# DavidHan008/SLAM-1

Hardware: AMD Instinct MI355X
Metric: frames/sec tracking+local-BA @1280x720 (higher is better)
Workload: dtype u8+f32+f64

## Files before the change

### include/slam355.h

```cpp
#ifndef SLAM355_H
#define SLAM355_H

#include <stddef.h>
#include <stdint.h>

#ifdef __cplusplus
extern "C" {
#endif

#define SLAM355_ABI_VERSION 1

#define SLAM_OK 0
#define SLAM_ERR_ARG (-1)
#define SLAM_ERR_HIP (-2)
#define SLAM_ERR_WORKSPACE (-3)
#define SLAM_ERR_COMM (-4)

int slam_abi_version(void);
const char* slam_last_error(void);
int slam_device_count(void);

int slam_hamming_knn2(const uint8_t* d_q, const int32_t* d_nq, int q_cap,
                      const uint8_t* d_t, const int32_t* d_nt, int t_cap,
                      int batch, int32_t* d_idx2, int32_t* d_dist2,
// ... 142 lines not shown
  double* delta_c;
  double* red_part;
  double* small;
  double* state;
  uint32_t* ticket;
  const int32_t* sg_ptr;
  const int32_t* sg_meta;
  const int32_t* obs_meta;
  const int32_t* chk_optr;
  const int32_t* chk_cptr;
  const int32_t* bslot_ab;
  const int32_t* tl_sched;
  const int32_t* tl_sched_host;
  int32_t* asm_tab;
  const int32_t* asm_act;
  int32_t n_asm_act;
  int32_t loss;
  double loss_scale;
  const uint32_t* cam_fixed;
} slam_ba_problem;
int slam_ba_problem_size(void);

#define SLAM_TL_FLOW_MAX_T 256

#ifndef SLAM_BA_MAX_BATCH
#define SLAM_BA_MAX_BATCH 16
#endif

enum {
  SLAM_PLAN_PERM = 0,
  SLAM_PLAN_ORDER,
  SLAM_PLAN_OBS_CAM, SLAM_PLAN_OBS_PT, SLAM_PLAN_PT_PTR, SLAM_PLAN_GRP_PTR,
  SLAM_PLAN_GRP_CSLOT, SLAM_PLAN_CSLOT_CAM, SLAM_PLAN_GRP_BSLOT, SLAM_PLAN_BSLOT_BLK,
  SLAM_PLAN_BLOCKS, SLAM_PLAN_CAM_CSLOT_PTR, SLAM_PLAN_CSLOT_ROW, SLAM_PLAN_BLK_BSLOT_PTR,
  SLAM_PLAN_BSLOT_ROW, SLAM_PLAN_SG_PTR, SLAM_PLAN_SG_META, SLAM_PLAN_SG_CAMS,
  SLAM_PLAN_OBS_LA, SLAM_PLAN_CHK_COBS, SLAM_PLAN_OBS_META, SLAM_PLAN_CHK_OPTR,
  SLAM_PLAN_CHK_CPTR, SLAM_PLAN_BSLOT_AB,
  SLAM_PLAN_NTAB
};
typedef struct slam_ba_plan_info {
  int32_t ok, n_obs, n_grps, n_sgrps, n_cslots, n_bslots, n_blocks, chunks_per_wg;
  long long off[SLAM_PLAN_NTAB], len[SLAM_PLAN_NTAB];
  long long total;
} slam_ba_plan_info;
long long slam_ba_plan_bound(int n_cams, int n_pts, int n_obs, int n_block_list);
int slam_ba_plan_mfma(int n_cams, int n_pts, int n_obs, const int32_t* cam_idx,
                      const int32_t* pt_idx, const int32_t* block_list, int n_block_list,
                      int chunks_per_wg, int32_t* out, long long out_cap,
                      slam_ba_plan_info* info);

#define SLAM_STAGE_NF64 17
#define SLAM_STAGE_META (12 + SLAM_STAGE_NF64 + SLAM_PLAN_NTAB)
int slam_ba_stage_windows(int n_win, int n, int cap, const double* rows, const int32_t* cnt,
                          const double* maps, int map_cap, const int32_t* M, const double* cams,
                          double u_off, double v_off, double* h64, long long cap64, int32_t* h32,
                          long long cap32, const void* d64, const void* d32,
                          slam_ba_problem* probs, long long* meta, long long* need);

int slam_ba_red_slots(int n_grps);
long long slam_ba_chol_len(int n_cams, const int32_t* tl_sched_host);
long long slam_ba_sys_len(int n_cams, int n_blocks);

int slam_ba_build_system(const slam_ba_problem* prob, void* stream);
int slam_ba_solve_step(const slam_ba_problem* prob, void* stream);
int slam_ba_decide(const slam_ba_problem* prob, void* stream);
int slam_ba_iterate(const slam_ba_problem* prob, int n_iter, void* stream);
int slam_ba_reset(const slam_ba_problem* prob, double lambda0, void* stream);
int slam_ba_iterate_batch(const slam_ba_problem* probs, int n_probs, int n_iter, void* stream);

long long slam_ba_cov_workspace_len(int n_cams);
int slam_ba_covariance(const slam_ba_problem* prob, const int32_t* d_pairs, int n_pairs,
                       double rank_tol, double* d_cov, double* d_ws, long long ws_len,
                       int32_t* d_status, void* stream);

int slam_ba_covariance_points(const slam_ba_problem* prob,
                              const int32_t* d_pairs, int n_pairs, double* d_cov,
                              const int32_t* d_points, int n_points, double* d_cov_pp,
                              const int32_t* d_cross, int n_cross, double* d_cov_pc,
                              double rank_tol, double* d_ws, long long ws_len,
                              int32_t* d_status , void* stream);

int slam_ba_set_solve_lds_floor(int bytes);

int slam_orb_set_lds_floor(int bytes);

int slam_orb_set_corner_cap(int entries_per_wave);

int slam_count_min(const int32_t* d_count, int n, int32_t* d_min, void* stream);
int slam_ba_reset_batch(const slam_ba_problem* probs, int n_probs, double lambda0, void* stream);

#define SLAM_COMM_ID_BYTES 128
typedef struct slam_comm_opaque* slam_comm_t;
int slam_comm_unique_id(void* h_id);
int slam_comm_init(int nranks, int rank, const void* h_id, slam_comm_t* comm);
int slam_comm_destroy(slam_comm_t comm);
int slam_comm_allreduce_f64(slam_comm_t comm, double* d_buf, long long n, void* stream);
int slam_ba_step_distributed(const slam_ba_problem* prob, slam_comm_t comm, void* stream);


int slam_pose_chain_objective(const double* params, int n_vec, int n_frames, int loop,
                              double* resid, void* stream);
long long slam_pose_chain_workspace_len(int n_frames);
int slam_pose_chain_trf(double* ws, int n_frames, int loop, int max_iter, int first, double ftol,
                        double xtol, double gtol, int max_nfev, double* state, void* stream);

typedef struct slam_pg_problem {
  int32_t n_poses, n_edges;
  int32_t loss;
  int32_t sched_len;
  double loss_scale;
  double* poses[2];
  const int32_t* edge_ij;
  const int32_t* edge_ij_host;
  const double* meas;
  const double* sqrt_info;
  const uint32_t* pose_fixed;
  const int32_t* sched;
  const int32_t* sched_host;
  double* ws;
  long long ws_len;
  double* state;
} slam_pg_problem;
int slam_pg_problem_size(void);
long long slam_pg_workspace_len(int n_poses, int n_edges, int n_tiles_stored);
int slam_pg_reset(const slam_pg_problem* prob, double lambda0, void* stream);
int slam_pg_iterate(const slam_pg_problem* prob, int n_iters, void* stream);
int slam_pg_residual(const slam_pg_problem* prob, double* d_e, double* d_r, void* stream);
int slam_pg_jacobian(const slam_pg_problem* prob, double* d_Ji, double* d_Jj, void* stream);

long long slam_pg_cov_workspace_len(int n_poses, int n_cols);
int slam_pg_covariance(const slam_pg_problem* prob, const int32_t* d_pairs, const int32_t* pairs_host,
                       int n_pairs, double rank_tol, double* d_cov ,
                       double* d_ws, long long ws_len, int32_t* d_status, void* stream);
int slam_pg_gate(const slam_pg_problem* prob, const int32_t* d_cand_ij, const int32_t* cand_ij_host,
                 const double* d_meas, const double* d_sqrt_info , int n_cand,
                 double rank_tol, double* d_d2, double* d_P, double* d_e ,
                 double* d_ws, long long ws_len, int32_t* d_status , void* stream);


int slam_bow_histograms(const uint8_t* desc, const int32_t* count, int n_each, int n_img, int cap,
                        const double* centers, int n_clusters, int32_t* labels, int32_t* hist,
                        void* stream);
int slam_bow_query(const int32_t* qhist, int n_query, const int32_t* db, const int32_t* n_db,
                   int n_clusters, int32_t* idx, double* val, void* stream);
int slam_bow_lloyd(const uint8_t* X, int n_points, double* centers, double* centers_tmp,
                   int n_clusters, int n_iter, int32_t* labels, double* shift, void* stream);


int slam_fast_tiles_workspace_bytes(int batch, int H, int W, int tile_h, int tile_w, int per_tile,
                                    size_t* bytes);
int slam_fast_tiles(const uint8_t* d_img, int batch, int H, int W, int stride, int tile_h,
                    int tile_w, int threshold, int per_tile, void* d_ws, size_t ws_bytes,
                    float* d_kp, int32_t* d_count, int kp_cap, void* stream);

int slam_lk_pyramid_layout(int H, int W, int win, int max_level, int* nlev, size_t* img_bytes);
int slam_lk_build_pyramids(const uint8_t* d_img, int n_img, int H, int W, int stride, int win,
                           int max_level, uint8_t* d_pyr, int16_t* d_deriv, void* stream);
int slam_lk_track(const uint8_t* d_prev_pyr, const int16_t* d_prev_deriv, const uint8_t* d_next_pyr,
                  long long pair_stride_imgs, int batch, int H, int W, int win, int max_level,
                  int max_count, double eps, float min_eig, const float* d_pts, int pts_stride,
                  const int32_t* d_npts, int cap, float* d_out, uint8_t* d_status, float* d_err,
                  void* stream);
int slam_lk_filter(const float* d_p1, int p1_stride, const float* d_p2, const uint8_t* d_status,
                   const float* d_err, const int32_t* d_npts, int cap, int batch, int H, int W,
                   float max_error, int lower_bounds, float* d_tp1, float* d_tp2, int32_t* d_idx,
                   int32_t* d_count, void* stream);
// ... 23 lines not shown
```

### slam-1_amd/csrc/ba.hip

```cpp
#include "ba_common.hpp"
#include "ba_epilogue.hpp"
#include "ba_layout.hpp"
#include "ba_project.hpp"
#include "dpp_fmac.hpp"

using slam::Launch;
using slam::launch_build;
using slam::make_launch;

namespace {

constexpr double kLamMin = 1e-16, kLamMax = 1e32;

#ifndef SLAM_BA_XCD
#define SLAM_BA_XCD 1
#endif
__device__ __forceinline__ int2 ba_xcd_map() {
  const int gx = (int)gridDim.x, n = (int)gridDim.y;
  if (!SLAM_BA_XCD || n < 8 || (n & 7)) return int2{(int)blockIdx.x, (int)blockIdx.y};
  const int lin = (int)blockIdx.y * gx + (int)blockIdx.x;
  const int xcd = lin & 7, slot = lin >> 3;
  const int wi = slot / gx;
  return int2{slot - wi * gx, xcd + 8 * wi};
}
// ... 1129 lines not shown
int check_problem(const slam_ba_problem* p) {
  SLAM_REQUIRE(p != nullptr, "slam_ba: null problem");
  SLAM_REQUIRE(p->n_cams > 0 && p->n_pts >= 0 && p->n_obs >= 0, "slam_ba: bad sizes");
  SLAM_REQUIRE(p->loss >= 0 && p->loss <= 3,
               "slam_ba: loss %d (0 linear, 1 huber, 2 soft_l1, 3 cauchy)", p->loss);
  SLAM_REQUIRE(p->loss == 0 || (std::isfinite(p->loss_scale) && p->loss_scale > 0.0),
               "slam_ba: loss %d needs a finite loss_scale > 0, not %g", p->loss, p->loss_scale);
  SLAM_REQUIRE(p->cams[0] && p->cams[1] && p->camrec[0] && p->camrec[1] &&
                   p->cpart && p->bpart && p->grp_ptr && p->grp_cslot && p->grp_bslot &&
                   p->cslot_obs_ptr && p->bslot_pair_ptr && p->cam_cslot_ptr && p->cslot_row && p->bslot_row &&
                   p->blk_bslot_ptr && p->blocks && p->ticket && p->sys && p->state &&
                   p->small && p->red_part && p->delta_c,
               "slam_ba: null buffer");
  SLAM_REQUIRE(p->n_grps >= 1, "slam_ba: n_grps must be >= 1 (an empty group for P = 0)");
  SLAM_REQUIRE(p->lin_mode == 0 || p->lin_mode == 1, "slam_ba: lin_mode must be 0 or 1");
  SLAM_REQUIRE(p->chk_optr != nullptr, "slam_ba: chk_optr (= pt_ptr[grp_ptr]) required");
  SLAM_REQUIRE(p->lin_mode == 0 || (p->n_sgrps >= 1 && p->sg_ptr && p->sg_meta && p->obs_meta &&
                                     p->chk_cptr && p->bslot_ab),
               "slam_ba: lin_mode 1 needs n_sgrps >= 1 and the supergroup tables");
  SLAM_REQUIRE(sys_packed(p->n_cams) ? (p->n_blocks >= p->n_cams &&
                                        p->n_blocks <= p->n_cams * (p->n_cams + 1) / 2)
                                     : p->n_blocks == p->n_cams * (p->n_cams + 1) / 2,
               "slam_ba: n_blocks must list all C(C+1)/2 upper blocks (9C <= %d) or the "
               "diagonal and every block with common points (packed)", kDenseMaxN);
  SLAM_REQUIRE(!p->tl_sched == !p->tl_sched_host,
               "slam_ba: tl_sched and tl_sched_host come together");
  SLAM_REQUIRE(p->asm_act == nullptr ||
                   (sys_packed(p->n_cams) && p->asm_tab == nullptr && p->n_asm_act >= 1 &&
                    p->n_asm_act <= p->n_blocks),
               "slam_ba: asm_act (n_asm_act %d of %d blocks) needs a packed system without asm_tab",
               p->n_asm_act, p->n_blocks);
  SLAM_REQUIRE(p->tl_mode == 0 || p->tl_mode == 1, "slam_ba: tl_mode must be 0 or 1");
  SLAM_REQUIRE(!sys_packed(p->n_cams) || p->chol != nullptr,
               "slam_ba: chol workspace (slam_ba_chol_len doubles) required for 9C > %d",
               kLdsMaxN);
  SLAM_REQUIRE(!sys_packed(p->n_cams) || p->tl_sched != nullptr,
               "slam_ba: the tile schedule (tl_sched, ba.tl_schedule) is required for 9C > %d",
               kLdsMaxN);
  return SLAM_OK;
}

}

extern "C" int slam_ba_red_slots(int n_grps) { return 2 * n_grps; }

extern "C" int slam_ba_problem_size(void) { return (int)sizeof(slam_ba_problem); }

extern "C" long long slam_ba_sys_len(int n_cams, int n_blocks) {
  const long long c9 = 9ll * n_cams;
  return sys_vec_off(n_cams, n_blocks) + 3 * c9 + n_cams;
}

extern "C" int slam_ba_residual(const double* d_cams, const double* d_pts,
                                const int32_t* d_cam_idx, const int32_t* d_pt_idx,
                                const double* d_qs, int n_obs, double* d_resid, void* stream) {
  SLAM_REQUIRE(n_obs >= 0, "slam_ba_residual: n_obs < 0");
  if (n_obs == 0) return SLAM_OK;
  SLAM_REQUIRE(d_cams && d_pts && d_cam_idx && d_pt_idx && d_qs && d_resid,
               "slam_ba_residual: null pointer");
  k_residual<<<nblk(n_obs, kBS), kBS, 0, slam::as_stream(stream)>>>(
      d_cams, d_pts, d_cam_idx, d_pt_idx, d_qs, n_obs, d_resid, nullptr);
  SLAM_LAUNCHED("k_residual");
  return SLAM_OK;
}

extern "C" int slam_ba_jacobian(const double* d_cams, const double* d_pts,
                                const int32_t* d_cam_idx, const int32_t* d_pt_idx,
                                const double* d_qs, int n_obs, double* d_resid, double* d_jac,
                                void* stream) {
  SLAM_REQUIRE(n_obs >= 0, "slam_ba_jacobian: n_obs < 0");
  if (n_obs == 0) return SLAM_OK;
  SLAM_REQUIRE(d_cams && d_pts && d_cam_idx && d_pt_idx && d_qs && d_resid && d_jac,
               "slam_ba_jacobian: null pointer");
  k_residual<<<nblk(n_obs, kBS), kBS, 0, slam::as_stream(stream)>>>(
      d_cams, d_pts, d_cam_idx, d_pt_idx, d_qs, n_obs, d_resid, d_jac);
  SLAM_LAUNCHED("k_residual(jac)");
  return SLAM_OK;
}

namespace {

static size_t g_solve_lds_floor = 0;

static int launch_reset(const Launch& L, double lam0, hipStream_t s) {
  k_reset<<<dim3(1, L.n), 64, 0, s>>>(L.b, lam0);
  SLAM_LAUNCHED("k_reset");
  return SLAM_OK;
}

}

int slam::make_launch(const slam_ba_problem* probs, int n, Launch* L) {
  SLAM_REQUIRE(n >= 1 && n <= kBaMaxBatch, "slam_ba: batch of %d problems (1..%d)", n, kBaMaxBatch);
  SLAM_REQUIRE(probs != nullptr, "slam_ba: null problem array");
  L->n = n;
  L->max_grps = L->max_blocks = L->max_sgrps = 0;
  L->mode = probs[0].lin_mode;
  L->solve_lds = 0;
  L->dense = true;
  L->robust = false;
  for (int i = 0; i < n; ++i) {
    if (int rc = check_problem(probs + i)) return rc;
    for (int j = 0; j < i; ++j)
      SLAM_REQUIRE(probs[j].state != probs[i].state && probs[j].sys != probs[i].sys,
                   "slam_ba: problems %d and %d of a batch share buffers", j, i);
    SLAM_REQUIRE(probs[i].lin_mode == L->mode,
                 "slam_ba: problems of one batch must share lin_mode");
    L->b.p[i] = probs[i];
    L->max_grps = max(L->max_grps, probs[i].n_grps);
    L->max_sgrps = max(L->max_sgrps, probs[i].n_sgrps);
    L->max_blocks = max(L->max_blocks, probs[i].asm_act != nullptr ? probs[i].n_asm_act : probs[i].n_blocks);
    L->solve_lds = std::max(L->solve_lds, slam::solve_blk_lds(probs[i].n_cams));
    L->solve_lds = std::max(L->solve_lds, g_solve_lds_floor);
    L->dense = L->dense && !sys_packed(probs[i].n_cams);
    L->robust = L->robust || probs[i].loss != 0;
  }
  SLAM_REQUIRE(n == 1 || L->dense,
               "slam_ba: batched problems must use the one-workgroup solver (9C <= %d)", kLdsMaxN);
  return SLAM_OK;
}

int slam::launch_build(const Launch& L, hipStream_t s) {
  bool folded = L.mode == 1;
  for (int i = 0; i < L.n; ++i) folded = folded && L.b.p[i].asm_tab != nullptr;
  if (L.mode == 1) {
    if (L.robust) k_lin_mfma<true><<<dim3(L.max_sgrps, L.n), kMWG, 0, s>>>(L.b);
    else k_lin_mfma<false><<<dim3(L.max_sgrps, L.n), kMWG, 0, s>>>(L.b);
    SLAM_LAUNCHED("k_lin_mfma");
  } else {
    if (L.robust) k_linearize<true><<<dim3(L.max_grps, L.n), kLinWG, 0, s>>>(L.b);
    else k_linearize<false><<<dim3(L.max_grps, L.n), kLinWG, 0, s>>>(L.b);
    SLAM_LAUNCHED("k_linearize");
  }
  if (!folded) {
    k_assemble<<<dim3(L.max_blocks, L.n), kAsmWG, 0, s>>>(L.b);
    SLAM_LAUNCHED("k_assemble");
  }
  return SLAM_OK;
}

namespace {

static int launch_solve(const Launch& L, bool fuse_decide, hipStream_t s) {
  if (int rc = L.dense ? slam::launch_solve_blk(L, s) : slam::launch_solve_tiled(L.b.p[0], s)) return rc;
  if (L.robust) {
    if (fuse_decide) k_back_trial<true, true><<<dim3(L.max_grps, L.n), kGrp, 0, s>>>(L.b);
    else k_back_trial<false, true><<<dim3(L.max_grps, L.n), kGrp, 0, s>>>(L.b);
  } else if (fuse_decide) {
    k_back_trial<true, false><<<dim3(L.max_grps, L.n), kGrp, 0, s>>>(L.b);
  } else {
    k_back_trial<false, false><<<dim3(L.max_grps, L.n), kGrp, 0, s>>>(L.b);
  }
  SLAM_LAUNCHED("k_back_trial");
  return SLAM_OK;
}

}

extern "C" int slam_ba_set_solve_lds_floor(int bytes) {
  SLAM_REQUIRE(bytes >= 0 && bytes <= 160 * 1024, "slam_ba_set_solve_lds_floor: %d B", bytes);
  g_solve_lds_floor = (size_t)bytes;
  return SLAM_OK;
}

extern "C" int slam_ba_reset(const slam_ba_problem* prob, double lambda0, void* stream) {
  return slam_ba_reset_batch(prob, 1, lambda0, stream);
}

extern "C" int slam_ba_reset_batch(const slam_ba_problem* probs, int n_probs, double lambda0,
                                   void* stream) {
  SLAM_REQUIRE(n_probs >= 0, "slam_ba_reset_batch: n_probs < 0");
  SLAM_REQUIRE(n_probs == 0 || probs != nullptr, "slam_ba_reset_batch: null problem array");
  for (int i0 = 0; i0 < n_probs; i0 += kBaMaxBatch) {
    Launch L;
    const int n = min(kBaMaxBatch, n_probs - i0);
    for (int i = 0; i < n; ++i)
      if (int rc = check_problem(probs + i0 + i)) return rc;
    L.n = n;
    for (int i = 0; i < n; ++i) L.b.p[i] = probs[i0 + i];
    if (int rc = launch_reset(L, lambda0, slam::as_stream(stream))) return rc;
  }
  return SLAM_OK;
}

extern "C" int slam_ba_build_system(const slam_ba_problem* prob, void* stream) {
  Launch L;
  if (int rc = make_launch(prob, 1, &L)) return rc;
  return launch_build(L, slam::as_stream(stream));
}

extern "C" int slam_ba_solve_step(const slam_ba_problem* prob, void* stream) {
  Launch L;
  if (int rc = make_launch(prob, 1, &L)) return rc;
  return launch_solve(L, false, slam::as_stream(stream));
}

extern "C" int slam_ba_decide(const slam_ba_problem* prob, void* stream) {
  Launch L;
  if (int rc = make_launch(prob, 1, &L)) return rc;
  k_decide<<<dim3(1, 1), 64, 0, slam::as_stream(stream)>>>(L.b);
  SLAM_LAUNCHED("k_decide");
  return SLAM_OK;
}

extern "C" int slam_ba_iterate(const slam_ba_problem* prob, int n_iter, void* stream) {
  return slam_ba_iterate_batch(prob, 1, n_iter, stream);
}

extern "C" int slam_ba_iterate_batch(const slam_ba_problem* probs, int n_probs, int n_iter,
                                     void* stream) {
  SLAM_REQUIRE(n_probs >= 0 && n_iter >= 0, "slam_ba_iterate_batch: negative count");
  SLAM_REQUIRE(n_probs == 0 || probs != nullptr, "slam_ba_iterate_batch: null problem array");
  hipStream_t s = slam::as_stream(stream);
  int i0 = 0;
  while (i0 < n_probs) {
    int n = 0;
    while (n < kBaMaxBatch && i0 + n < n_probs && (n == 0 || !sys_packed(probs[i0 + n].n_cams)) &&
           !(n > 0 && sys_packed(probs[i0].n_cams)))
      ++n;
    Launch L;
    if (int rc = make_launch(probs + i0, n, &L)) return rc;
    for (int it = 0; it < n_iter; ++it) {
      if (int rc = launch_build(L, s)) return rc;
      if (int rc = launch_solve(L, true, s)) return rc;
    }
    i0 += n;
  }
  return SLAM_OK;
}

#ifdef SLAM_LINM_PROFILE
extern "C" int slam_linm_stamps(unsigned long long* out, int n) {
  SLAM_HIP(hipDeviceSynchronize());
  SLAM_HIP(hipMemcpyFromSymbol(out, HIP_SYMBOL(g_linm_stamp), (size_t)n * 8 * sizeof(unsigned long long)));
  return SLAM_OK;
}
#endif
```

### slam-1_amd/csrc/ba_common.hpp

```cpp
#pragma once

#include "common.hpp"

#include <cmath>

namespace {

typedef double d4 __attribute__((ext_vector_type(4)));

constexpr double kDiagMin = 1e-6, kDiagMax = 1e32;

constexpr int kBaMaxBatch = SLAM_BA_MAX_BATCH;
struct BaBatch {
  slam_ba_problem p[kBaMaxBatch];
};
#define BA_PROB(b) const slam_ba_problem& p = (b).p[blockIdx.y]
static_assert(sizeof(slam_ba_problem) == 408, "slam_ba_problem grew: re-check the kernarg size");
static_assert(sizeof(BaBatch) <= 16 * 408, "BaBatch kernel argument size");

__device__ __forceinline__ void lm_wave_priority() { __builtin_amdgcn_s_setprio(3); }

__device__ __forceinline__ double block_sum(double v, double* lds) {
  for (int off = 32; off > 0; off >>= 1) v += __shfl_down(v, off, 64);
  const int lane = threadIdx.x & 63, wid = threadIdx.x >> 6;
  if (lane == 0) lds[wid] = v;
  __syncthreads();
  double s = 0.0;
  if (threadIdx.x == 0) {
    const int nw = (blockDim.x + 63) >> 6;
    for (int w = 0; w < nw; ++w) s += lds[w];
  }
  __syncthreads();
  return s;
}

__device__ __forceinline__ int cur_of(const double* state) {
  return state[SLAM_BA_ST_CUR] != 0.0 ? 1 : 0;
}

__device__ __forceinline__ double clampd(double d) { return fmin(fmax(d, kDiagMin), kDiagMax); }

constexpr int kDenseMaxN = 120;
__host__ __device__ __forceinline__ bool sys_packed(int n_cams) { return 9 * n_cams > kDenseMaxN; }
__host__ __device__ __forceinline__ long long sys_vec_off(int n_cams, int n_blocks) {
  return sys_packed(n_cams) ? 81ll * n_blocks : 81ll * n_cams * n_cams;
}
constexpr int kLdsMaxN = kDenseMaxN;

__device__ __forceinline__ void st_sc1(double* p, double v) {
  __hip_atomic_store(p, v, __ATOMIC_RELAXED, __HIP_MEMORY_SCOPE_AGENT);
}
__device__ __forceinline__ double ld_sc1(const double* p) {
  return __hip_atomic_load(const_cast<double*>(p), __ATOMIC_RELAXED, __HIP_MEMORY_SCOPE_AGENT);
}
__device__ __forceinline__ unsigned ticket_add(uint32_t* p) {
  return __hip_atomic_fetch_add(p, 1u, __ATOMIC_RELAXED, __HIP_MEMORY_SCOPE_AGENT);
}
__device__ __forceinline__ void ticket_reset(uint32_t* p) {
  __hip_atomic_store(p, 0u, __ATOMIC_RELAXED, __HIP_MEMORY_SCOPE_AGENT);
}

constexpr int kBS = 256;

}

namespace slam {

struct Launch {
  BaBatch b;
  int n, max_grps, max_blocks, max_sgrps, mode;
  size_t solve_lds;
  bool dense;
  bool robust;
};

size_t solve_blk_lds(int n_cams);
int launch_solve_blk(const Launch& L, hipStream_t s);
int launch_solve_tiled(const slam_ba_problem& p, hipStream_t s);
int make_launch(const slam_ba_problem* probs, int n, Launch* L);
int launch_build(const Launch& L, hipStream_t s);

}
```

### slam-1_amd/csrc/ba_solve.hip

```cpp
#include "ba_common.hpp"
#include "ba_epilogue.hpp"
#include "dpp_fmac.hpp"

namespace {

constexpr int kSolveHdr = 32;

#ifdef SLAM_SOLVE_PROFILE
#define SOLVE_PROF_T(i) uint64_t prof_t##i = wall_clock64()
#define SOLVE_PROF_END()                                                        \
  do {                                                                          \
    const uint64_t prof_e = wall_clock64();                                     \
    if (threadIdx.x == 0) {                                                     \
      p.state[12] = 10.0 * (double)(prof_t1 - prof_t0);                         \
      p.state[13] = 10.0 * (double)(prof_t2 - prof_t1);                         \
      p.state[14] = 10.0 * (double)(prof_t3 - prof_t2);                         \
      p.state[15] = 10.0 * (double)(prof_e - prof_t3);                          \
    }                                                                           \
  } while (0)
#else
#define SOLVE_PROF_T(i) (void)0
#define SOLVE_PROF_END() (void)0
#endif

constexpr int kBlkWG = 256;
constexpr int kBlkWaves = kBlkWG / 64;
constexpr int kTileMax = 9;
constexpr int kPanelW = 9;
constexpr int kWLs = 13;
static_assert(kLdsMaxN <= kBlkWG, "k_solve_blk prefetch assumes one element per thread");
static_assert(kBlkWaves * kTileMax >= ((kLdsMaxN + 16) / 16) * ((kLdsMaxN + 16) / 16 + 1) / 2,
              "kTileMax too small");

__device__ __forceinline__ double rcp_f64(double d) {
  double r = __builtin_amdgcn_rcp(d);
  double e = __builtin_fma(-d, r, 1.0);
  r = __builtin_fma(r, e, r);
  e = __builtin_fma(-d, r, 1.0);
  return __builtin_fma(r, e, r);
}

__device__ __forceinline__ double readlane_d(double v, int lane) {
  const unsigned long long u = (unsigned long long)__double_as_longlong(v);
  const unsigned lo = (unsigned)__builtin_amdgcn_readlane((int)(unsigned)u, lane);
  const unsigned hi = (unsigned)__builtin_amdgcn_readlane((int)(unsigned)(u >> 32), lane);
  return __longlong_as_double((long long)(((unsigned long long)hi << 32) | lo));
}

struct BlkLds {
  int n16;
  int pn, wl, ll, lf, dd, yy, xx, ep, total;
  __host__ __device__ explicit BlkLds(int n) {
    n16 = ((n + 1 + 15) / 16) * 16;
    pn = kSolveHdr;
    wl = pn + n16 * kPanelW;
    ll = wl + n16 * kWLs;
    lf = ll + n16 * kWLs;
    dd = lf + ((n * (n - 1) / 2 + 1) & ~1);
    yy = dd + ((n + 1) & ~1);
    xx = yy + ((n + 1) & ~1);
    ep = xx + ((n + 1) & ~1);
    total = ep + 5 * ((n + 1) & ~1);
  }
};

#ifdef SLAM_SOLVE_TRACE
__device__ unsigned long long g_solve_trace[20][6];
#define SOLVE_TR(step, i)                                                        \
  do {                                                                           \
    if (threadIdx.x == 0 && blockIdx.y == 0 && (step) < 20)                      \
      g_solve_trace[step][i] = __builtin_amdgcn_s_memtime();                     \
  } while (0)
#else
#define SOLVE_TR(step, i) (void)0
#endif

__global__ __launch_bounds__(kBlkWG) __attribute__((amdgpu_waves_per_eu(2))) void k_solve_blk(BaBatch bat) {
  BA_PROB(bat);
  lm_wave_priority();
  extern __shared__ __attribute__((aligned(16))) double lds[];
  double* red = lds;
  int* fail_p = reinterpret_cast<int*>(lds + 16);
  const int n = 9 * p.n_cams;
  const BlkLds g(n);
  double* Pn = lds + g.pn;
  double* WL = lds + g.wl;
  double* LL = lds + g.ll;
  double* LF = lds + g.lf;
  double* Dd = lds + g.dd;
  double* Yy = lds + g.yy;
  double* X = lds + g.xx;
  const double* S = p.sys;
  const double* bvec = S + (size_t)n * n;
  const double* diagU = bvec + 2 * n;
  const double lam = p.state[SLAM_BA_ST_LAMBDA];
  const int t = threadIdx.x, lane = t & 63;
  const int wid = __builtin_amdgcn_readfirstlane(t >> 6);
  const int NT = g.n16 / 16, NL = NT * (NT + 1) / 2;
  SOLVE_PROF_T(0);
  SOLVE_TR(19, 1);
  const int n2 = (n + 1) & ~1;
  if (t == 0) *fail_p = 0;
  for (int i = t; i < 2 * g.n16 * kWLs; i += kBlkWG) WL[i] = 0.0;
  int tI[kTileMax], tJ[kTileMax];
  d4 acc[kTileMax];
#pragma unroll
  for (int s = 0; s < kTileMax; ++s) {
    const int tl = wid + kBlkWaves * s;
    int I = 0;
    while ((I + 1) * (I + 2) / 2 <= tl) ++I;
    tI[s] = tl < NL ? I : -1;
    tJ[s] = tl < NL ? tl - I * (I + 1) / 2 : -1;
    const int col = min(max(tJ[s], 0) * 16 + (lane & 15), n - 1);
#pragma unroll
    for (int q = 0; q < 4; ++q) {
      const int row = min(max(tI[s], 0) * 16 + (lane >> 4) + 4 * q, n - 1);
      acc[s][q] = S[(size_t)row * n + col];
    }
  }
  double* Eb = lds + g.ep;
  {
    const double* src[5] = {bvec, bvec + n, diagU, p.cams[cur_of(p.state)], diagU + n};
    const int len[5] = {n, n, n, n, p.n_cams};
    double v[5];
#pragma unroll
    for (int a = 0; a < 5; ++a) v[a] = src[a][min(t, len[a] - 1)];
#pragma unroll
    for (int a = 0; a < 5; ++a)
      if (t < len[a]) Eb[a * n2 + t] = v[a];
  }
  __syncthreads();
#pragma unroll
  for (int s = 0; s < kTileMax; ++s) {
    const int col = tJ[s] * 16 + (lane & 15);
#pragma unroll
    for (int q = 0; q < 4; ++q) {
      const int row = tI[s] * 16 + (lane >> 4) + 4 * q;
      double a = acc[s][q];
      if (row == col) a += lam * clampd(Eb[2 * n2 + col]);
      if (row == n) a = Eb[min(col, n - 1)];
      if (tI[s] < 0 || col >= n || row > n) a = 0.0;
      acc[s][q] = a;
    }
  }
  SOLVE_PROF_T(1);
  bool ok = true;
  SOLVE_TR(19, 0);
  for (int c0 = 0; c0 < n; c0 += kPanelW) {
    SOLVE_TR(c0 / kPanelW, 0);
#pragma unroll
    for (int s = 0; s < kTileMax; ++s) {
      if (tI[s] < 0 || tJ[s] * 16 + 15 < c0 || tJ[s] * 16 >= c0 + kPanelW || tI[s] * 16 + 15 < c0)
        continue;
      const int col = tJ[s] * 16 + (lane & 15);
#pragma unroll
      for (int q = 0; q < 4; ++q) {
        const int row = tI[s] * 16 + (lane >> 4) + 4 * q;
        if (col >= c0 && col < c0 + kPanelW && col <= row && row >= c0 && row <= n)
          Pn[(row - c0) * kPanelW + (col - c0)] = acc[s][q];
      }
    }
    __syncthreads();
    SOLVE_TR(c0 / kPanelW, 1);
    constexpr int kRowsBelow = 16 - kPanelW;
    const int nbelow = n + 1 - c0 - kPanelW;
    const int nw = max(1, (nbelow + 4 * kRowsBelow - 1) / (4 * kRowsBelow));
    if (wid < nw) {
      const int rl = lane & 15, rg = lane >> 4;
      const bool piv = rl < kPanelW;
      const int r = piv ? c0 + rl
                        : c0 + kPanelW + 4 * kRowsBelow * wid + kRowsBelow * rg + (rl - kPanelW);
      const bool valid = r <= n;
      const double* pr = Pn + (r - c0) * kPanelW;
      double u[kPanelW];
#pragma unroll
      for (int j = 0; j < kPanelW; ++j) u[j] = valid && (!piv || j <= rl) ? pr[j] : 0.0;
      double Dinv[kPanelW];
      bool bad = false;
      static_for<0, kPanelW>([&](auto J) {
        constexpr int j = decltype(J)::value;
        const double d = bcast16<j>(u[j]);
        bad |= !(d > 0.0) || !isfinite(d);
        Dinv[j] = rcp_f64(d);
        const double l = u[j] * Dinv[j];
        if constexpr (j + 1 < kPanelW) u[j + 1] = __builtin_fma(-l, bcast16<j + 1>(u[j]), u[j + 1]);
        static_assert(kPanelW == 9, "the BcastFmaTail ranges of dpp_fmac.hpp end at row 8");
        BcastFmaTail<j + 2, kPanelW - 1>::run(u, u[j], -l);
      });
      if (valid && ((wid == 0 && rg == 0) || !piv)) {
        double* wl = WL + r * kWLs;
        double* ll = LL + r * kWLs;
        double* lf = LF + r * (r - 1) / 2 + c0;
        double lj[kPanelW];
#pragma unroll
        for (int j = 0; j < kPanelW; ++j) {
          lj[j] = u[j] * Dinv[j];
          wl[j] = -u[j];
          ll[j] = lj[j];
        }
        if (r == n) {
#pragma unroll
          for (int j = 0; j < kPanelW; ++j) Yy[c0 + j] = u[j];
        } else if (!piv) {
#pragma unroll
          for (int j = 0; j < kPanelW; ++j) lf[j] = lj[j];
        } else {
          double dm = u[0];
#pragma unroll
          for (int j = 1; j < kPanelW; ++j) dm = j == rl ? u[j] : dm;
          Dd[r] = dm;
#pragma unroll
          for (int j = 0; j < kPanelW - 1; ++j)
            if (j < rl) lf[j] = lj[j];
        }
// ... 14 lines not shown
      const double* wrow = WL + (tI[s] * 16 + (lane & 15)) * kWLs + (lane >> 4);
      const double* lrow = LL + (tJ[s] * 16 + (lane & 15)) * kWLs + (lane >> 4);
      double wa[3], lb[3];
#pragma unroll
      for (int kk = 0; kk < 3; ++kk) {
        wa[kk] = wrow[4 * kk];
        lb[kk] = lrow[4 * kk];
      }
#pragma unroll
      for (int kk = 0; kk < 3; ++kk)
        acc[s] = __builtin_amdgcn_mfma_f64_16x16x4f64(wa[kk], lb[kk], acc[s], 0, 0, 0);
    }
#ifdef SLAM_SOLVE_TRACE
    if (threadIdx.x == 0) {
      double chk = acc[0][0];
      __asm__ volatile("" : "+v"(chk));
      acc[0][0] = chk;
    }
    SOLVE_TR(c0 / kPanelW, 4);
#endif
  }
  SOLVE_PROF_T(2);
  SOLVE_TR(18, 0);
  if (ok && wid == 0) {
    double x0 = lane < n ? Yy[lane] / Dd[lane] : 0.0;
    double x1 = lane + 64 < n ? Yy[lane + 64] / Dd[lane + 64] : 0.0;
    constexpr int kBackU = 8;
    int k = n - 1;
    for (; k - kBackU + 1 >= 64; k -= kBackU) {
      double l0[kBackU], l1[kBackU];
#pragma unroll
      for (int u = 0; u < kBackU; ++u) {
        const int kk = k - u;
        const double* Lk = LF + kk * (kk - 1) / 2;
        l0[u] = Lk[lane];
        const double v = Lk[min(lane + 64, kk - 1)];
        l1[u] = lane + 64 < kk ? v : 0.0;
      }
#pragma unroll
      for (int u = 0; u < kBackU; ++u) {
        const double xk = readlane_d(x1, k - u - 64);
        x0 = __builtin_fma(-l0[u], xk, x0);
        x1 = __builtin_fma(-l1[u], xk, x1);
      }
    }
    for (; k >= 64; --k) {
      const double* Lk = LF + k * (k - 1) / 2;
      const double v = Lk[min(lane + 64, k - 1)];
      const double xk = readlane_d(x1, k - 64);
      x0 = __builtin_fma(-Lk[lane], xk, x0);
      x1 = __builtin_fma(-(lane + 64 < k ? v : 0.0), xk, x1);
    }
    for (; k - kBackU + 1 >= 1; k -= kBackU) {
      double l0[kBackU];
#pragma unroll
      for (int u = 0; u < kBackU; ++u) {
        const int kk = k - u;
        const double v = LF[kk * (kk - 1) / 2 + min(lane, kk - 1)];
        l0[u] = lane < kk ? v : 0.0;
      }
#pragma unroll
      for (int u = 0; u < kBackU; ++u) x0 = __builtin_fma(-l0[u], readlane_d(x0, k - u), x0);
    }
    for (; k >= 1; --k) {
      const double v = LF[k * (k - 1) / 2 + min(lane, k - 1)];
      x0 = __builtin_fma(-(lane < k ? v : 0.0), readlane_d(x0, k), x0);
    }
    if (lane < n) X[lane] = x0;
    if (lane + 64 < n) X[lane + 64] = x1;
  }
  __syncthreads();
  SOLVE_PROF_T(3);
  SOLVE_TR(18, 1);
  solve_epilogue(p, X, ok, red, EpiSrc{Eb + n2, Eb + 2 * n2, Eb + 3 * n2, Eb + 4 * n2});
  SOLVE_PROF_END();
  SOLVE_TR(18, 2);
}

}

size_t slam::solve_blk_lds(int n_cams) { return sizeof(double) * BlkLds(9 * n_cams).total; }

int slam::launch_solve_blk(const Launch& L, hipStream_t s) {
  k_solve_blk<<<dim3(1, L.n), kBlkWG, L.solve_lds, s>>>(L.b);
  SLAM_LAUNCHED("k_solve_blk");
  return SLAM_OK;
}

#ifdef SLAM_SOLVE_TRACE
extern "C" int slam_solve_trace(unsigned long long* out) {
  SLAM_HIP(hipDeviceSynchronize());
  SLAM_HIP(hipMemcpyFromSymbol(out, HIP_SYMBOL(g_solve_trace), 20 * 6 * sizeof(unsigned long long)));
  return SLAM_OK;
}
#endif
```

### slam-1_amd/slam355/_lib.py

```python
from __future__ import annotations

import ctypes
import os

_HERE = os.path.dirname(os.path.abspath(__file__))
LIB_PATH = os.environ.get("SLAM355_LIB") or os.path.join(_HERE, "libslam355.so")

c_int = ctypes.c_int
c_double = ctypes.c_double
c_size_t = ctypes.c_size_t
c_p = ctypes.c_void_p
c_uint64 = ctypes.c_uint64
c_longlong = ctypes.c_longlong

c_i32 = ctypes.c_int32


class BAProblemStruct(ctypes.Structure):
    _fields_ = [
        ("n_cams", c_i32), ("n_pts", c_i32), ("n_obs", c_i32), ("n_grps", c_i32),
        ("n_blocks", c_i32), ("n_cslots", c_i32), ("n_bslots", c_i32), ("lin_mode", c_i32),
        ("n_sgrps", c_i32), ("tl_mode", c_i32),
        ("cams", c_p * 2), ("pts", c_p * 2), ("camrec", c_p * 2),
        ("obs_cam", c_p), ("obs_pt", c_p), ("obs_q", c_p), ("pt_ptr", c_p), ("grp_ptr", c_p),
# ... 14 lines not shown


class PGProblemStruct(ctypes.Structure):
    _fields_ = [
        ("n_poses", c_i32), ("n_edges", c_i32), ("loss", c_i32), ("sched_len", c_i32),
        ("loss_scale", ctypes.c_double), ("poses", c_p * 2),
        ("edge_ij", c_p), ("edge_ij_host", c_p), ("meas", c_p), ("sqrt_info", c_p),
        ("pose_fixed", c_p), ("sched", c_p), ("sched_host", c_p),
        ("ws", c_p), ("ws_len", ctypes.c_longlong), ("state", c_p),
    ]


_PG = ctypes.POINTER(PGProblemStruct)

PLAN_TABLES = ("perm", "order", "obs_cam", "obs_pt", "pt_ptr", "grp_ptr", "grp_cslot", "cslot_cam",
               "grp_bslot", "bslot_blk", "blocks", "cam_cslot_ptr", "cslot_row", "blk_bslot_ptr",
               "bslot_row", "sg_ptr", "sg_meta", "sg_cams", "obs_la", "chk_cobs", "obs_meta",
               "chk_optr", "chk_cptr", "bslot_ab")


class PlanInfo(ctypes.Structure):
    _fields_ = [
        ("ok", c_i32), ("n_obs", c_i32), ("n_grps", c_i32), ("n_sgrps", c_i32),
        ("n_cslots", c_i32), ("n_bslots", c_i32), ("n_blocks", c_i32), ("chunks_per_wg", c_i32),
        ("off", ctypes.c_longlong * len(PLAN_TABLES)), ("len", ctypes.c_longlong * len(PLAN_TABLES)),
        ("total", ctypes.c_longlong),
    ]

SIGNATURES = {
    "slam_abi_version": [],
    "slam_last_error": [],
    "slam_device_count": [],
    "slam_hamming_knn2": [c_p, c_p, c_int, c_p, c_p, c_int, c_int, c_p, c_p, c_p, c_p],
    "slam_compact_matches": [c_p, c_p, c_p, c_int, c_int, c_p, c_double, c_p, c_p, c_p],
    "slam_orb_workspace_bytes": [c_int, c_int, c_int, c_int, c_int, c_int, c_int,
                                 ctypes.POINTER(c_size_t)],
    "slam_orb_tiles": [c_p, c_int, c_int, c_int, c_int, c_int, c_int, c_int, c_int, c_p,
                       c_size_t, c_p, c_p, c_p, c_p, c_int, c_p],
    "slam_gather_matches": [c_p, c_int, c_p, c_int, c_p, c_p, c_p, c_p, c_int, c_int, c_p, c_p,
                            c_p, c_p, c_p],
    "slam_gather_temporal": [c_p, c_p, c_int, c_p, c_int, c_p, c_p, c_int, c_int, c_p, c_p, c_p,
                             c_p],
    "slam_triangulate": [c_p, c_p, c_p, c_int, c_int, c_p, c_p, c_int, c_p, c_p],
    "slam_pnp_ransac": [c_p, c_p, c_p, c_int, c_int, c_p, c_uint64, c_int, c_int, c_double, c_int,
                        c_int, c_p, c_p, c_p, c_p, c_p, c_longlong, c_p],
    "slam_pnp_workspace_len": [c_int, c_int],
    "slam_pnp_ransac_ws": [c_p, c_p, c_p, c_int, c_int, c_p, c_uint64, c_int, c_int, c_double,
                           c_int, c_int, c_p, c_p, c_p, c_p, c_p, c_longlong, c_p, c_longlong, c_p],
    "slam_pnp_scratch_len": [c_int, c_int],
    "slam_pose_chain": [c_p, c_p, c_p, c_int, c_p, c_p, c_p],
    "slam_vo_estimate_pose": [c_p, c_p, c_p, c_p, c_p, c_int, c_int, c_p, c_uint64, c_int, c_int,
                              c_int, c_int, c_p, c_p, c_p, c_p, c_p, c_size_t, c_p],
    "slam_vo_pose_workspace_bytes": [c_int, c_int, ctypes.POINTER(c_size_t)],
    "slam_vo_residuals": [c_p, c_p, c_p, c_p, c_p, c_p, c_int, c_int, c_p, c_p, c_p],
    "slam_map_workspace_bytes": [c_int, c_int, ctypes.POINTER(c_size_t)],
    "slam_rel_to_abs": [c_p, c_p, c_int, c_int, c_p, c_p, c_p],
    "slam_map_windows": [c_p, c_p, c_int, c_int, c_int, c_p, c_p, c_p, c_p, c_int, c_double, c_p,
                         c_p, c_size_t, c_p],
    "slam_map_associate": [c_p, c_p, c_int, c_int, c_p, c_p, c_p, c_p, c_int, c_double, c_int,
                           c_p, c_p, c_size_t, c_p],
    "slam_fundamental_lmeds": [c_p, c_p, c_p, c_int, c_int, c_uint64, c_int, c_int, c_p, c_p, c_p,
                               c_p],
    "slam_fundamental_lmeds_ws": [c_p, c_p, c_p, c_int, c_int, c_uint64, c_int, c_int, c_p, c_p,
                                  c_p, c_p, c_longlong, c_p],
    "slam_fundamental_workspace_len": [c_int, c_int],
    "slam_filter_pairs": [c_p, c_p, c_p, c_int, c_int, c_p, c_p, c_p],
    "slam_ba_residual": [c_p, c_p, c_p, c_p, c_p, c_int, c_p, c_p],
    "slam_ba_jacobian": [c_p, c_p, c_p, c_p, c_p, c_int, c_p, c_p, c_p],
    "slam_ba_red_slots": [c_int],
    "slam_ba_problem_size": [],
    "slam_ba_sys_len": [c_int, c_int],
    "slam_ba_chol_len": [c_int, c_p],
    "slam_ba_build_system": [_PROB, c_p],
    "slam_ba_solve_step": [_PROB, c_p],
    "slam_ba_decide": [_PROB, c_p],
    "slam_ba_iterate": [_PROB, c_int, c_p],
    "slam_ba_reset": [_PROB, c_double, c_p],
    "slam_ba_iterate_batch": [_PROB, c_int, c_int, c_p],
    "slam_ba_cov_workspace_len": [c_int],
    "slam_ba_covariance": [_PROB, c_p, c_int, c_double, c_p, c_p, c_longlong, c_p, c_p],
    "slam_ba_covariance_points": [_PROB, c_p, c_int, c_p, c_p, c_int, c_p, c_p, c_int, c_p, c_double, c_p,
                                  c_longlong, c_p, c_p],
    "slam_ba_set_solve_lds_floor": [c_int],
    "slam_orb_set_lds_floor": [c_int],
    "slam_orb_set_corner_cap": [c_int],
    "slam_count_min": [c_p, c_int, c_p, c_p],
    "slam_hamming_force_valu": [c_int],
    "slam_ba_reset_batch": [_PROB, c_int, c_double, c_p],
    "slam_pose_chain_objective": [c_p, c_int, c_int, c_int, c_p, c_p],
    "slam_bow_histograms": [c_p, c_p, c_int, c_int, c_int, c_p, c_int, c_p, c_p, c_p],
    "slam_bow_query": [c_p, c_int, c_p, c_p, c_int, c_p, c_p, c_p],
    "slam_bow_lloyd": [c_p, c_int, c_p, c_p, c_int, c_int, c_p, c_p, c_p],
    "slam_pose_chain_workspace_len": [c_int],
    "slam_pg_problem_size": [],
    "slam_pg_workspace_len": [c_int, c_int, c_int],
    "slam_pg_reset": [_PG, c_double, c_p],
    "slam_pg_iterate": [_PG, c_int, c_p],
    "slam_pg_residual": [_PG, c_p, c_p, c_p],
    "slam_pg_jacobian": [_PG, c_p, c_p, c_p],
    "slam_pg_cov_workspace_len": [c_int, c_int],
    "slam_pg_covariance": [_PG, c_p, c_p, c_int, c_double, c_p, c_p, c_longlong, c_p, c_p],
    "slam_pg_gate": [_PG, c_p, c_p, c_p, c_p, c_int, c_double, c_p, c_p, c_p, c_p, c_longlong, c_p, c_p],
    "slam_fast_tiles_workspace_bytes": [c_int, c_int, c_int, c_int, c_int, c_int,
                                        ctypes.POINTER(c_size_t)],
    "slam_fast_tiles": [c_p, c_int, c_int, c_int, c_int, c_int, c_int, c_int, c_int, c_p,
                        c_size_t, c_p, c_p, c_int, c_p],
    "slam_lk_pyramid_layout": [c_int, c_int, c_int, c_int, ctypes.POINTER(c_int),
                               ctypes.POINTER(c_size_t)],
    "slam_lk_build_pyramids": [c_p, c_int, c_int, c_int, c_int, c_int, c_int, c_p, c_p, c_p],
    "slam_lk_track": [c_p, c_p, c_p, ctypes.c_longlong, c_int, c_int, c_int, c_int, c_int, c_int,
                      c_double, ctypes.c_float, c_p, c_int, c_p, c_int, c_p, c_p, c_p, c_p],
    "slam_lk_filter": [c_p, c_int, c_p, c_p, c_p, c_p, c_int, c_int, c_int, c_int, ctypes.c_float,
                       c_int, c_p, c_p, c_p, c_p, c_p],
    "slam_sgbm_workspace_bytes": [c_int, c_int, c_int, c_int, c_int, c_int,
                                  ctypes.POINTER(c_size_t)],
    "slam_sgbm": [c_p, c_p, c_int, c_int, c_int, c_int, c_int, c_int, c_int, c_int, c_int, c_p,
                  c_size_t, c_p, c_p, c_p],
    "slam_vo_right_qs_3d": [c_p, c_p, c_p, c_int, c_int, c_p, ctypes.c_longlong,
                            ctypes.c_longlong, c_int, c_int, ctypes.c_float, ctypes.c_float, c_p,
                            c_p, c_p, c_p, c_p, c_p, c_p, c_p, c_p, c_p, c_p, c_p, c_p, c_p],
    "slam_triangulate_f32": [c_p, c_p, c_p, c_int, c_int, c_p, c_p, c_p, c_p],
    "slam_pose_chain_trf": [c_p, c_int, c_int, c_int, c_int, c_double, c_double, c_double, c_int,
                            c_p, c_p],
    "slam_comm_unique_id": [c_p],
    "slam_comm_init": [c_int, c_int, c_p, ctypes.POINTER(c_p)],
    "slam_comm_destroy": [c_p],
    "slam_comm_allreduce_f64": [c_p, c_p, ctypes.c_longlong, c_p],
    "slam_ba_step_distributed": [_PROB, c_p, c_p],
    "slam_ba_plan_bound": [c_int, c_int, c_int, c_int],
    "slam_ba_plan_mfma": [c_int, c_int, c_int, c_p, c_p, c_p, c_int, c_int, c_p, c_longlong,
                          ctypes.POINTER(PlanInfo)],
    "slam_ba_stage_windows": [c_int, c_int, c_int, c_p, c_p, c_p, c_int, c_p, c_p, c_double,
                              c_double, c_p, c_longlong, c_p, c_longlong, c_p, c_p, c_p, c_p, c_p],
}
_RESTYPE = {"slam_last_error": ctypes.c_char_p, "slam_ba_sys_len": ctypes.c_longlong,
            "slam_ba_plan_bound": ctypes.c_longlong,
            "slam_ba_chol_len": ctypes.c_longlong, "slam_ba_cov_workspace_len": ctypes.c_longlong,
            "slam_pnp_workspace_len": ctypes.c_longlong,
            "slam_pnp_scratch_len": ctypes.c_longlong,
            "slam_fundamental_workspace_len": ctypes.c_longlong,
            "slam_pose_chain_workspace_len": ctypes.c_longlong,
            "slam_pg_workspace_len": ctypes.c_longlong,
            "slam_pg_cov_workspace_len": ctypes.c_longlong}


class SlamError(RuntimeError):
    """A libslam355 call returned a non-zero status."""


def _load():
    if not os.path.exists(LIB_PATH):
        raise ImportError(
            f"libslam355.so not found at {LIB_PATH}: build it with "
            "`make -C slam-1_amd` (or __graft_entry__.build()). slam355 has no CPU fallback."
        )
    import torch

    lib = ctypes.CDLL(LIB_PATH)
    for name, argtypes in SIGNATURES.items():
        fn = getattr(lib, name)
        fn.argtypes = argtypes
        fn.restype = _RESTYPE.get(name, c_int)
    return lib


lib = _load()
# ... 11 lines not shown
```

Before: 23980.

## Fuse Schur-block assembly into the one-workgroup dense solve kernel

```diff
diff --git a/include/slam355.h b/include/slam355.h
--- a/include/slam355.h
+++ b/include/slam355.h
@@ -248,6 +248,8 @@
 
 int slam_ba_set_solve_lds_floor(int bytes);
 
+int slam_ba_set_fused_assembly(int on);
+
 int slam_orb_set_lds_floor(int bytes);
 
 int slam_orb_set_corner_cap(int entries_per_wave);
diff --git a/slam-1_amd/csrc/ba.hip b/slam-1_amd/csrc/ba.hip
--- a/slam-1_amd/csrc/ba.hip
+++ b/slam-1_amd/csrc/ba.hip
@@ -1235,6 +1235,9 @@
 
 static size_t g_solve_lds_floor = 0;
 
+static int g_fused_assembly = 1;
+constexpr int kFuseMaxRows = 1024;
+
 static int launch_reset(const Launch& L, double lam0, hipStream_t s) {
   k_reset<<<dim3(1, L.n), 64, 0, s>>>(L.b, lam0);
   SLAM_LAUNCHED("k_reset");
@@ -1252,6 +1255,7 @@
   L->solve_lds = 0;
   L->dense = true;
   L->robust = false;
+  L->fused = false;
   for (int i = 0; i < n; ++i) {
     if (int rc = check_problem(probs + i)) return rc;
     for (int j = 0; j < i; ++j)
@@ -1285,7 +1289,7 @@
     else k_linearize<false><<<dim3(L.max_grps, L.n), kLinWG, 0, s>>>(L.b);
     SLAM_LAUNCHED("k_linearize");
   }
-  if (!folded) {
+  if (!folded && !L.fused) {
     k_assemble<<<dim3(L.max_blocks, L.n), kAsmWG, 0, s>>>(L.b);
     SLAM_LAUNCHED("k_assemble");
   }
@@ -1313,6 +1317,12 @@
 extern "C" int slam_ba_set_solve_lds_floor(int bytes) {
   SLAM_REQUIRE(bytes >= 0 && bytes <= 160 * 1024, "slam_ba_set_solve_lds_floor: %d B", bytes);
   g_solve_lds_floor = (size_t)bytes;
+  return SLAM_OK;
+}
+
+extern "C" int slam_ba_set_fused_assembly(int on) {
+  SLAM_REQUIRE(on >= 0 && on <= 2, "slam_ba_set_fused_assembly: %d (0, 1 or 2)", on);
+  g_fused_assembly = on;
   return SLAM_OK;
 }
 
@@ -1373,6 +1383,12 @@
       ++n;
     Launch L;
     if (int rc = make_launch(probs + i0, n, &L)) return rc;
+    L.fused = g_fused_assembly != 0 && L.dense;
+    for (int i = 0; i < n; ++i) {
+      const slam_ba_problem& q = probs[i0 + i];
+      L.fused = L.fused && q.asm_tab == nullptr && q.asm_act == nullptr &&
+                (g_fused_assembly == 2 || q.n_cslots + q.n_bslots <= kFuseMaxRows);
+    }
     for (int it = 0; it < n_iter; ++it) {
       if (int rc = launch_build(L, s)) return rc;
       if (int rc = launch_solve(L, true, s)) return rc;
diff --git a/slam-1_amd/csrc/ba_common.hpp b/slam-1_amd/csrc/ba_common.hpp
--- a/slam-1_amd/csrc/ba_common.hpp
+++ b/slam-1_amd/csrc/ba_common.hpp
@@ -72,6 +72,7 @@
   size_t solve_lds;
   bool dense;
   bool robust;
+  bool fused;
 };
 
 size_t solve_blk_lds(int n_cams);
diff --git a/slam-1_amd/csrc/ba_solve.hip b/slam-1_amd/csrc/ba_solve.hip
--- a/slam-1_amd/csrc/ba_solve.hip
+++ b/slam-1_amd/csrc/ba_solve.hip
@@ -16,6 +16,7 @@
       p.state[13] = 10.0 * (double)(prof_t2 - prof_t1);                         \
       p.state[14] = 10.0 * (double)(prof_t3 - prof_t2);                         \
       p.state[15] = 10.0 * (double)(prof_e - prof_t3);                          \
+      p.state[17] = 10.0 * (double)(prof_ta - prof_t0);                         \
     }                                                                           \
   } while (0)
 #else
@@ -75,6 +76,166 @@
 #define SOLVE_TR(step, i) (void)0
 #endif
 
+constexpr int kAsmVirt = 1024;
+constexpr int kAsmNF = 8;
+constexpr int kAsmGrp = 3;
+
+template <int N>
+__device__ __forceinline__ double asm_pair_sum(const double* a) {
+  if constexpr (N == 1) return a[0];
+  else return asm_pair_sum<N / 2>(a) + asm_pair_sum<N / 2>(a + N / 2);
+}
+
+template <int N, int HOIST>
+__device__ __forceinline__ void virt_rows_sum2(const double* __restrict__ part, int stride, int rb,
+                                               int re, int lane, double& o0, double& o1) {
+  constexpr int P = kAsmVirt / N;
+  static_assert(HOIST <= kAsmNF, "hoisted rows of a part: one accumulator each");
+  const double* q0 = part + (size_t)rb * stride + lane;
+  const double* q1 = part + (size_t)rb * stride + min(lane + 64, N - 1);
+  const int R = re - rb;
+  double v0 = 0.0, v1 = 0.0;
+  if (R <= HOIST * P) {
+    double x0[HOIST * P], x1[HOIST * P];
+#pragma unroll
+    for (int i = 0; i < HOIST * P; ++i) {
+      x0[i] = 0.0;
+      x1[i] = 0.0;
+      if (i < R) {
+        x0[i] = q0[(size_t)i * stride];
+        x1[i] = q1[(size_t)i * stride];
+      }
+    }
+#pragma unroll
+    for (int k = 0; k < P; ++k) {
+      double a0[kAsmNF] = {}, a1[kAsmNF] = {};
+#pragma unroll
+      for (int u = 0; u < HOIST; ++u) {
+        a0[u] += x0[k + u * P];
+        a1[u] += x1[k + u * P];
+      }
+      v0 += asm_pair_sum<kAsmNF>(a0);
+      v1 += asm_pair_sum<kAsmNF>(a1);
+    }
+  } else {
+    static_assert(P % kAsmGrp == 0, "parts walked in groups");
+    const int trips = ((R + P - 1) / P + kAsmNF - 1) / kAsmNF;
+#pragma unroll 1
+    for (int k0 = 0; k0 < P; k0 += kAsmGrp) {
+      double a0[kAsmGrp][kAsmNF] = {}, a1[kAsmGrp][kAsmNF] = {};
+#pragma unroll 1
+      for (int m = 0; m < trips; ++m) {
+        double y0[kAsmGrp][kAsmNF], y1[kAsmGrp][kAsmNF];
+#pragma unroll
+        for (int g = 0; g < kAsmGrp; ++g)
+#pragma unroll
+          for (int u = 0; u < kAsmNF; ++u) {
+            const int r = k0 + g + (u + kAsmNF * m) * P;
+            y0[g][u] = 0.0;
+            y1[g][u] = 0.0;
+            if (r < R) {
+              y0[g][u] = q0[(size_t)r * stride];
+              y1[g][u] = q1[(size_t)r * stride];
+            }
+          }
+#pragma unroll
+        for (int g = 0; g < kAsmGrp; ++g)
+#pragma unroll
+          for (int u = 0; u < kAsmNF; ++u) {
+            a0[g][u] += y0[g][u];
+            a1[g][u] += y1[g][u];
+          }
+      }
+#pragma unroll
+      for (int g = 0; g < kAsmGrp; ++g) {
+        v0 += asm_pair_sum<kAsmNF>(a0[g]);
+        v1 += asm_pair_sum<kAsmNF>(a1[g]);
+      }
+    }
+  }
+  o0 = v0;
+  o1 = v1;
+}
+
+constexpr bool asm_stage_fits() {
+  for (int c = 1; 9 * c <= kLdsMaxN; ++c) {
+    const int n = 9 * c, n16 = ((n + 1 + 15) / 16) * 16, nt = n16 / 16;
+    if (nt * (nt + 1) / 2 * 256 > n16 * (kPanelW + 2 * kWLs) + n * (n - 1) / 2) return false;
+  }
+  return true;
+}
+static_assert(asm_stage_fits(), "k_solve_blk<true>: the tile staging overruns Pn / WL / LL / LF");
+
+__device__ __forceinline__ void asm_prologue(const slam_ba_problem& p, double* stg, double* Eb,
+                                             int n2, int wid, int lane) {
+  const int C9 = 9 * p.n_cams;
+  double* S = p.sys;
+  double* bvec = S + sys_vec_off(p.n_cams, p.n_blocks);
+  double* gvec = bvec + C9;
+  double* diagU = gvec + C9;
+  double* costc = diagU + C9;
+  auto put = [&](int row, int col, double v) {
+    S[(size_t)row * C9 + col] = v;
+    const int I = row >> 4, J = col >> 4;
+    if (I >= J) stg[(I * (I + 1) / 2 + J) * 256 + (row & 15) * 16 + (col & 15)] = v;
+  };
+  for (int blk = wid; blk < p.n_blocks; blk += kBlkWaves) {
+    const int c1 = p.blocks[2 * blk], c2 = p.blocks[2 * blk + 1];
+    const bool diag = c1 == c2;
+    const int bb = p.blk_bslot_ptr[blk], be = p.blk_bslot_ptr[blk + 1];
+    const int t0 = lane, t1 = min(lane + 64, 80);
+    const bool has1 = lane + 64 < 81;
+    const int i0 = t0 / 9, j0 = t0 - 9 * i0, i1 = t1 / 9, j1 = t1 - 9 * i1;
+    if (!diag && be == bb) {
+      put(9 * c1 + i0, 9 * c2 + j0, -0.0);
+      put(9 * c2 + j0, 9 * c1 + i0, -0.0);
+      if (has1) {
+        put(9 * c1 + i1, 9 * c2 + j1, -0.0);
+        put(9 * c2 + j1, 9 * c1 + i1, -0.0);
+      }
+      continue;
+    }
+    double sh0 = 0.0, sh1 = 0.0, sb0 = 0.0, sb1 = 0.0;
+    if (diag)
+      virt_rows_sum2<109, 4>(p.cpart, kCPart, p.cam_cslot_ptr[c1], p.cam_cslot_ptr[c1 + 1], lane, sh0, sh1);
+    if (!diag || be > bb) virt_rows_sum2<81, 3>(p.bpart, 81, bb, be, lane, sb0, sb1);
+    if (diag) {
+      const int s0 = 9 * j0 + i0, s1 = 9 * j1 + i1;
+      const double a0 = __shfl(sb0, s0 & 63, 64), b0 = __shfl(sb1, s0 & 63, 64);
+      const double a1 = __shfl(sb0, s1 & 63, 64), b1 = __shfl(sb1, s1 & 63, 64);
+      const double sbT0 = s0 < 64 ? a0 : b0, sbT1 = s1 < 64 ? a1 : b1;
+      const double shu = __shfl(sh1, (lane + 9) & 63, 64);
+      put(9 * c1 + i0, 9 * c1 + j0, sh0 - (sb0 + sbT0));
+      if (has1) put(9 * c1 + i1, 9 * c1 + j1, sh1 - (sb1 + sbT1));
+      const int e = lane + 64;
+      if (e >= 81 && e < 90) {
+        const int q = 9 * c1 + e - 81;
+        const double gv = -sh1, bv = -sh1 - shu;
+        gvec[q] = gv;
+        bvec[q] = bv;
+        Eb[n2 + q] = gv;
+        Eb[q] = bv;
+      }
+      if (e >= 99 && e < 108) {
+        diagU[9 * c1 + e - 99] = sh1;
+        Eb[2 * n2 + 9 * c1 + e - 99] = sh1;
+      }
+      if (e == 108) {
+        costc[c1] = sh1;
+        Eb[4 * n2 + c1] = sh1;
+      }
+    } else {
+      put(9 * c1 + i0, 9 * c2 + j0, -sb0);
+      put(9 * c2 + j0, 9 * c1 + i0, -sb0);
+      if (has1) {
+        put(9 * c1 + i1, 9 * c2 + j1, -sb1);
+        put(9 * c2 + j1, 9 * c1 + i1, -sb1);
+      }
+    }
+  }
+}
+
+template <bool ASM>
 __global__ __launch_bounds__(kBlkWG) __attribute__((amdgpu_waves_per_eu(2))) void k_solve_blk(BaBatch bat) {
   BA_PROB(bat);
   lm_wave_priority();
@@ -101,7 +262,16 @@
   SOLVE_TR(19, 1);
   const int n2 = (n + 1) & ~1;
   if (t == 0) *fail_p = 0;
-  for (int i = t; i < 2 * g.n16 * kWLs; i += kBlkWG) WL[i] = 0.0;
+  if constexpr (!ASM)
+    for (int i = t; i < 2 * g.n16 * kWLs; i += kBlkWG) WL[i] = 0.0;
+  if constexpr (ASM) {
+    double* Ea = lds + g.ep;
+    asm_prologue(p, Pn, Ea, n2, wid, lane);
+    const double cv = p.cams[cur_of(p.state)][min(t, n - 1)];
+    if (t < n) Ea[3 * n2 + t] = cv;
+    __syncthreads();
+  }
+  SOLVE_PROF_T(a);
   int tI[kTileMax], tJ[kTileMax];
   d4 acc[kTileMax];
 #pragma unroll
@@ -115,11 +285,15 @@
 #pragma unroll
     for (int q = 0; q < 4; ++q) {
       const int row = min(max(tI[s], 0) * 16 + (lane >> 4) + 4 * q, n - 1);
-      acc[s][q] = S[(size_t)row * n + col];
+      if constexpr (ASM) acc[s][q] = Pn[(tl < NL ? tl : 0) * 256 + ((lane >> 4) + 4 * q) * 16 + (lane & 15)];
+      else acc[s][q] = S[(size_t)row * n + col];
     }
   }
   double* Eb = lds + g.ep;
-  {
+  if constexpr (ASM) {
+    __syncthreads();
+    for (int i = t; i < 2 * g.n16 * kWLs; i += kBlkWG) WL[i] = 0.0;
+  } else {
     const double* src[5] = {bvec, bvec + n, diagU, p.cams[cur_of(p.state)], diagU + n};
     const int len[5] = {n, n, n, n, p.n_cams};
     double v[5];
@@ -128,8 +302,8 @@
 #pragma unroll
     for (int a = 0; a < 5; ++a)
       if (t < len[a]) Eb[a * n2 + t] = v[a];
-  }
-  __syncthreads();
+    __syncthreads();
+  }
 #pragma unroll
   for (int s = 0; s < kTileMax; ++s) {
     const int col = tJ[s] * 16 + (lane & 15);
@@ -310,7 +484,8 @@
 size_t slam::solve_blk_lds(int n_cams) { return sizeof(double) * BlkLds(9 * n_cams).total; }
 
 int slam::launch_solve_blk(const Launch& L, hipStream_t s) {
-  k_solve_blk<<<dim3(1, L.n), kBlkWG, L.solve_lds, s>>>(L.b);
+  if (L.fused) k_solve_blk<true><<<dim3(1, L.n), kBlkWG, L.solve_lds, s>>>(L.b);
+  else k_solve_blk<false><<<dim3(1, L.n), kBlkWG, L.solve_lds, s>>>(L.b);
   SLAM_LAUNCHED("k_solve_blk");
   return SLAM_OK;
 }
diff --git a/slam-1_amd/slam355/_lib.py b/slam-1_amd/slam355/_lib.py
--- a/slam-1_amd/slam355/_lib.py
+++ b/slam-1_amd/slam355/_lib.py
@@ -120,6 +120,7 @@
     "slam_ba_covariance_points": [_PROB, c_p, c_int, c_p, c_p, c_int, c_p, c_p, c_int, c_p, c_double, c_p,
                                   c_longlong, c_p, c_p],
     "slam_ba_set_solve_lds_floor": [c_int],
+    "slam_ba_set_fused_assembly": [c_int],
     "slam_orb_set_lds_floor": [c_int],
     "slam_orb_set_corner_cap": [c_int],
     "slam_count_min": [c_p, c_int, c_p, c_p],
```

After: 24660 (median of 6 runs). +2.9%, better.
